# lupoglaz/DeepLocalProteinDocking

Hardware: AMD Instinct MI355X
Metric: pose correlations/sec (48ch x 64^3 pair, 6-degree SOI-sized generated rotation set) (higher is better)
Workload: dtype f32

## Files before the change

### deeplocalproteindocking_amd/csrc/dlpd_k3r.hip

```cpp
#include <dlpd_platform.h>
#include "dlpd_fft.h"
#include "dlpd_internal.h"
#include "dlpd_k3.h"

template <int N> DLPD_D void init_twiddles_k3r(cplx* tw, int tid, int nthreads) {
  for (int k = tid; k < N; k += nthreads) {
    double s, c;
    sincospi(-2.0 * (double)k / (double)N, &s, &c);
    tw[k] = c_make((float)c, (float)s);
  }
}

#ifndef DLPD_K3R_F128
#define DLPD_K3R_F128 4
#endif
#ifndef DLPD_K3R_M160
#define DLPD_K3R_M160 10
#endif
#ifndef DLPD_K3R_TY160
#define DLPD_K3R_TY160 16
#endif
#ifndef DLPD_K3R_PBUF160W
#define DLPD_K3R_PBUF160W 2
#endif
#ifndef DLPD_K3R_DMA_BEHIND_LOADS
#define DLPD_K3R_DMA_BEHIND_LOADS 1
#endif
#ifndef DLPD_K3R_TWREG128
#define DLPD_K3R_TWREG128 1
#endif
#ifndef DLPD_K3R_PBUF128W
#define DLPD_K3R_PBUF128W 2
#endif
#ifndef DLPD_K3R_PBUF128
#define DLPD_K3R_PBUF128 1
#endif
#ifndef DLPD_K3R_PBUF160
#define DLPD_K3R_PBUF160 2
#endif
#ifndef DLPD_K3R_RAWBUF128
#define DLPD_K3R_RAWBUF128 1
#endif
#ifndef DLPD_K3R_FFT_PRIO
#define DLPD_K3R_FFT_PRIO 0
#endif
template <int N> struct K3rWideAbove { static constexpr int value = (N == 160) ? 24 : 32; };
template <int N, bool WIDE> struct K3rCfg;
template <> struct K3rCfg<64, false> { static constexpr int F = 4, M = 4, TY = 16, RAWBUF = 2, PBUF = 1; };
template <> struct K3rCfg<80, false> { static constexpr int F = 5, M = 5, TY = 16, RAWBUF = 2, PBUF = 1; };
template <> struct K3rCfg<128, false> { static constexpr int F = DLPD_K3R_F128, M = 8, TY = 16, RAWBUF = DLPD_K3R_RAWBUF128, PBUF = DLPD_K3R_PBUF128; };
template <> struct K3rCfg<160, false> { static constexpr int F = 5, M = DLPD_K3R_M160, TY = DLPD_K3R_TY160, RAWBUF = 1, PBUF = DLPD_K3R_PBUF160; };
template <> struct K3rCfg<80, true> { static constexpr int F = 5, M = 10, TY = 16, RAWBUF = 1, PBUF = 1; };
template <> struct K3rCfg<128, true> { static constexpr int F = 4, M = 8, TY = 8, RAWBUF = 1, PBUF = DLPD_K3R_PBUF128W; };
template <> struct K3rCfg<160, true> { static constexpr int F = 5, M = 10, TY = 8, RAWBUF = 1, PBUF = DLPD_K3R_PBUF160W; };

#ifdef DLPD_STAMPS
__device__ unsigned long long dlpd_stamps_k3r[32];
extern "C" int dlpd_debug_read_stamps_k3r(unsigned long long* host32) {
  if (hipMemcpyFromSymbol(host32, HIP_SYMBOL(dlpd_stamps_k3r), 32 * sizeof(unsigned long long)) != hipSuccess) return 1;
  unsigned long long z[32] = {0};
  return hipMemcpyToSymbol(HIP_SYMBOL(dlpd_stamps_k3r), z, sizeof(z)) == hipSuccess ? 0 : 1;
}
#endif

#ifndef DLPD_K3R_DC_OPAQUE
#define DLPD_K3R_DC_OPAQUE 0
#endif
#if defined(DLPD_CPU_EMU)
#define DLPD_K3R_KEEP4(q) ((void)0)
#else
#define DLPD_K3R_KEEP4(q) asm("" : "+v"((q).x), "+v"((q).y), "+v"((q).z), "+v"((q).w))
#endif
template <int NPAIR> DLPD_HD int k3r_pair_swz(int k) { return NPAIR == 8 ? ((k & 2) << 1) : 0; }

template <int N> struct K3rFirst { typedef FftPassW<N, N / 8, 1, +1, 8> Pass; };
template <int N, int NPAIR> DLPD_D void k3r_first_pass_load(typename K3rFirst<N>::Pass& ps, int t, int m, const float4* rj) {
  constexpr int NH = N / 2, R1 = N / 8, RH = R1 / 2;
  static_assert(NH % 8 == 0 && R1 % 2 == 0, "bins t + 8r: the first R1/2 direct, the others mirrored");
  const float4* lo = rj + NPAIR * t + (m ^ k3r_pair_swz<NPAIR>(t));
  const float4* hi = rj + NPAIR * (NH - t) + (m ^ k3r_pair_swz<NPAIR>(NH - t));
  {
    float4 q[RH];
#pragma unroll
    for (int r = 0; r < RH; r++) q[r] = lo[NPAIR * 8 * r];
    if (DLPD_K3R_DC_OPAQUE) DLPD_K3R_KEEP4(q[0]);
#pragma unroll
    for (int r = 0; r < RH; r++) {
      const bool dc = (r == 0) && (t == 0);
      ps.v[0][r] = dc ? c_make(q[r].x, q[r].z) : c_make(q[r].x - q[r].w, q[r].y + q[r].z);
    }
  }
  {
    float4 q[RH];
#pragma unroll
    for (int s = 0; s < RH; s++) q[s] = *(hi - NPAIR * 8 * s);
    if (DLPD_K3R_DC_OPAQUE) DLPD_K3R_KEEP4(q[0]);
#pragma unroll
    for (int s = 0; s < RH; s++) {
      const bool ny = (s == 0) && (t == 0);
      ps.v[0][RH + s] = ny ? c_make(q[s].x, q[s].z) : c_make(q[s].x + q[s].w, q[s].z - q[s].y);
    }
  }
  SmallDft<R1, +1>::run(ps.v[0]);
}
template <int N> DLPD_D void k3r_first_pass_store(cplx* S, int rowoff, int t, const typename K3rFirst<N>::Pass& ps) {
  constexpr int R1 = N / 8;
  cplx* P = S + rowoff;
  if constexpr (N == 160) {
#pragma unroll
    for (int r = 0; r < R1; r++) lds_st(P + 21 * t + r, ps.v[0][r]);
  } else if constexpr (N == 80) {
    const RowMid<R1 + 1> md = {rowoff};
    ps.store_blk(S, md, t);
  } else {
    const RowAddr<0> ad = {rowoff};
    ps.store(S, ad, t);
  }
}
template <int N, int NPAIR> DLPD_D void k3r_first_pass(cplx* S, int rowoff, int t, int m, const float4* rj) {
  typename K3rFirst<N>::Pass ps;
  k3r_first_pass_load<N, NPAIR>(ps, t, m, rj);
  k3r_first_pass_store<N>(S, rowoff, t, ps);
}

template <int N> struct K3rTwReg { static constexpr bool value = (N == 128) && (DLPD_K3R_TWREG128 != 0); };
template <int N> struct K3rSecond { typedef FftPassW<N, 8, N / 8, +1, 8> Pass; };
template <int N> DLPD_D void k3r_second_pass(cplx* S, int rowoff, int t, const cplx* tw,
                                             const cplx (&twr)[K3rSecond<N>::Pass::PER][7]) {
  constexpr int R1 = N / 8;
  DLPD_WAVE_SYNC();
  if constexpr (K3rTwReg<N>::value) {
    const RowAddr<0> ad = {rowoff};
    typename K3rSecond<N>::Pass ps;
    ps.load_twr(S, ad, t, twr);
    DLPD_WAVE_SYNC();
    ps.store(S, ad, t);
  } else if constexpr (N == 160) {
    cplx* P = S + rowoff;
    FftPassW<N, 8, 20, +1, 8> ps;
#pragma unroll
    for (int i = 0; i < 3; i++)
      if (t + 8 * i < 20) {
#pragma unroll
        for (int r = 0; r < 8; r++) ps.v[i][r] = lds_ld(P + t + 8 * i + 21 * r);
        ps.twiddle_and_run(i, t + 8 * i, tw);
      }
    DLPD_WAVE_SYNC();
#pragma unroll
    for (int i = 0; i < 3; i++)
      if (t + 8 * i < 20) {
#pragma unroll
        for (int r = 0; r < 8; r++) lds_st(P + t + 8 * i + 21 * r, ps.v[i][r]);
      }
  } else {
    const RowAddr<0> ad = {rowoff};
    FftPassW<N, 8, R1, +1, 8> ps;
    if constexpr (N == 80) {
      const RowMid<R1 + 1> md = {rowoff};
      ps.load_blk(S, md, t, tw);
    } else {
      ps.load(S, ad, t, tw);
    }
    DLPD_WAVE_SYNC();
    ps.store(S, ad, t);
  }
}

template <int N, int HP, int MODE> __global__ void __launch_bounds__(64 * (K3rCfg<N, (HP > K3rWideAbove<N>::value)>::F + K3rCfg<N, (HP > K3rWideAbove<N>::value)>::M))
k_zifft_filter_rs(const cplx* __restrict__ Bw, float* __restrict__ out, int CT, int C, int has_clash, int G,
                  const float* __restrict__ W1t, const float* __restrict__ b1, const float* __restrict__ W2,
                  float b2, int has_clip, float clip, float thr, K3Aux aux, int ntiles, int tpb, K3Cand cd) {
  typedef K3rCfg<N, (HP > K3rWideAbove<N>::value)> Cfg;
  constexpr int F = Cfg::F, M = Cfg::M, TY = Cfg::TY, RAWBUF = Cfg::RAWBUF;
  constexpr int NZ = N / 2 + 1, RS = N + 8, NPAIR = TY / 2, NYT = N / TY;
  constexpr int CPW = 8 / NPAIR;
  constexpr int LPK = 64 / NPAIR;
  constexpr int NFULL = (N / 2) / LPK;
  constexpr int GMAX = F * CPW;
  constexpr int NTM = 64 * M;
  constexpr int EPT = (NPAIR * N) / NTM;
  constexpr int MSTEP = NTM / N;
  constexpr int PBUF = Cfg::PBUF;
  constexpr int PSZ = F * 8 * RS;
  constexpr int RAWC = (PBUF == 2) ? NZ * NPAIR : ((NZ * NPAIR + 63) / 64) * 64;
  static_assert(NPAIR == 8 || NPAIR == 4, "one transform wave = 8 pencils x 8 threads");
  static_assert(EPT >= 1 && EPT * NTM == NPAIR * N && NTM % N == 0, "the filter waves tile the voxels exactly");
  static_assert(NZ * NPAIR == NFULL * 64 + NPAIR, "raw channel = NFULL full DMA instructions + one short one");
  DLPD_DYN_SHARED(cplx, S);
  cplx* tw = S + PBUF * PSZ;
  float4* raw = reinterpret_cast<float4*>(tw + N);
  const int tid = threadIdx.x, lane = tid & 63, wave = tid >> 6;
  const bool is_fft = wave < F;
  const int twave = wave, fwave = wave - F;
  const int t_beg = blockIdx.x * tpb, t_end = (t_beg + tpb < ntiles) ? t_beg + tpb : ntiles;
  if (t_beg >= t_end) return;
  const int plane = t_beg / NYT, plane_x = plane % N, plane_b = plane / N;
  init_twiddles_k3r<N>(tw, tid, 64 * (F + M));
  const unsigned cand_tau = (MODE == 1 && cd.keys) ? *cd.tau : 0u;
  const float clampv = has_clip ? clip : __builtin_inff();

  float4* rawg = raw + twave * CPW * RAWC;
  auto issue_channel = [&](int t, int cb, int buf, int lane) {
    const int ty0 = (t - plane * NYT) * TY, txo = plane_x, tb = plane_b;
#pragma unroll
    for (int j = 0; j < CPW; j++) {
      const int g = twave * CPW + j;
      if (g < G && cb + g < CT) {
        const cplx* src = Bw + (((size_t)tb * CT + cb + DLPD_UNIFORM(g)) * NZ * N + txo) * N + ty0;
        const unsigned lane_off = (unsigned)(((lane / NPAIR) * N * N + 2 * ((lane % NPAIR) ^ k3r_pair_swz<NPAIR>(lane / NPAIR))) * sizeof(cplx));
        const dlpd_lds_t rj = DLPD_LDS_ADDR(rawg + buf * (F * CPW * RAWC) + j * RAWC);
#pragma unroll
        for (int it = 0; it < NFULL; it++) DLPD_GLDS16_SOA(src + (size_t)it * LPK * N * N, lane_off, rj + it * 1024);
        const int mt = lane % NPAIR;
        if (PBUF == 1 || lane < NPAIR) DLPD_GLDS16_SOA(src + (size_t)(N / 2) * N * N, 2 * mt * sizeof(cplx), rj + NFULL * 1024);
      }
    }
  };
  const int tm = 64 * fwave + lane;
  const int zz_ = is_fft ? 0 : tm % N, m0_ = is_fft ? 0 : tm / N;

  if (is_fft) {
    if (DLPD_K3R_FFT_PRIO) DLPD_SET_PRIO(DLPD_K3R_FFT_PRIO);
    issue_channel(t_beg, 0, 0, lane);
  }
  DLPD_LDS_BARRIER();
  DLPD_STAMP_DECL;
  const int ngroups = (CT + G - 1) / G;
  const int nsteps = (t_end - t_beg) * ngroups;
  if (is_fft) {
    int t = t_beg, cbase = 0, rb = 0;
    cplx* P = S;
    cplx twr[K3rSecond<N>::Pass::PER][7];
    if constexpr (K3rTwReg<N>::value) {
      typename K3rSecond<N>::Pass ps0;
      ps0.fetch_twiddles(lane & 7, tw, twr);
    }
#pragma unroll 1
    for (int step = 0; step < nsteps; step++) {
      const int gn = (CT - cbase) < G ? (CT - cbase) : G;
      const bool last_group = cbase + G >= CT;
      const bool mine = twave * CPW < gn;
      int ln = lane;
      if (F + M > 12) DLPD_OPAQUE_V(ln);
      const int tr = ln & 7, qr = ln >> 3;
      if (mine) {
        DLPD_WAIT_VMEM();
        DLPD_WAVE_SYNC();
      }
      DLPD_STAMP(0);
      const int nt = last_group ? t + 1 : t, ncb = last_group ? 0 : cbase + G;
      if (RAWBUF == 2 && nt < t_end) issue_channel(nt, ncb, rb ^ 1, ln);
      if (mine) {
        const int m = qr % NPAIR, j = qr / NPAIR;
        k3r_first_pass<N, NPAIR>(P, (twave * 8 + qr) * RS, tr, m, rawg + rb * (F * CPW * RAWC) + j * RAWC);
        DLPD_WAVE_SYNC();
      }
      DLPD_STAMP(1);
      if constexpr (K3rTwReg<N>::value && DLPD_K3R_DMA_BEHIND_LOADS) {
        const RowAddr<0> ad = {(twave * 8 + qr) * RS};
        typename K3rSecond<N>::Pass ps;
        DLPD_WAVE_SYNC();
        if (mine) ps.load_only(P, ad, tr);
        if (RAWBUF == 1 && nt < t_end) issue_channel(nt, ncb, 0, ln);
        if (mine) {
          ps.run_twr(tr, twr);
          DLPD_WAVE_SYNC();
          ps.store(P, ad, tr);
        }
      } else {
        if (RAWBUF == 1 && nt < t_end) issue_channel(nt, ncb, 0, ln);
        if (mine) k3r_second_pass<N>(P, (twave * 8 + qr) * RS, tr, tw, twr);
      }
      DLPD_STAMP(2);
      if (RAWBUF == 2) rb ^= 1;
      DLPD_LDS_BARRIER();
      DLPD_STAMP(3);
      if (PBUF == 2) {
        P = (P == S) ? S + PSZ : S;
      } else {
        DLPD_LDS_BARRIER();
      }
      DLPD_STAMP(4);
      if (last_group) { cbase = 0; t++; } else cbase += G;
    }
  } else {
    float nrm[EPT * 2];
    float h[EPT * 2][HP];
    cplx vals[PBUF == 2 ? 1 : GMAX][EPT] = {};
    const cplx* P = S;
    int t = t_beg, cbase = 0;
#pragma unroll 1
    for (int step = 0; step < nsteps; step++) {
      const int y0 = (t - plane * NYT) * TY, xo = plane_x, b = plane_b;
      const int gn = (CT - cbase) < G ? (CT - cbase) : G;
      const bool last_group = cbase + G >= CT;
      int zz = zz_, m0 = m0_;
      DLPD_OPAQUE_V(zz);
      DLPD_OPAQUE_V(m0);
      if (cbase == 0) {
        if (MODE == 1 && cd.keys && !cand_tau && tm == 0) cd.count[cd.nb + b] = 1u;
#pragma unroll
        for (int e = 0; e < EPT * 2; e++) nrm[e] = 0.f;
        if (MODE == 1 && aux.C > 0) {
          const int Na = aux.N;
          size_t cstride = (size_t)Na * Na * Na;
          DLPD_OPAQUE_S(cstride);
          const float* ub = aux.p + (size_t)b * HP * cstride + ((size_t)(xo >> 1) * Na + (y0 >> 1)) * Na;
          unsigned lo[EPT];
#pragma unroll
          for (int e = 0; e < EPT; e++) lo[e] = (unsigned)((m0 + e * MSTEP) * Na + (zz >> 1));
#pragma unroll
          for (int e = 0; e < EPT; e++)
#pragma unroll
            for (int j = 0; j < HP; j++) {
              const float v = (ub + (size_t)j * cstride)[lo[e]];
              h[2 * e][j] = v;
              h[2 * e + 1][j] = v;
            }
        } else {
#pragma unroll
          for (int e = 0; e < EPT * 2; e++)
#pragma unroll
            for (int j = 0; j < HP; j++) h[e][j] = b1[j];
        }
      }
      DLPD_STAMP(0);
      DLPD_LDS_BARRIER();
      DLPD_STAMP(1);
      const int gs = (cbase + gn <= C) ? gn : (C - cbase > 0 ? C - cbase : 0);
      if (PBUF == 1) {
#pragma unroll
        for (int g = 0; g < GMAX; g++)
          if (g < gs) {
#pragma unroll
            for (int e = 0; e < EPT; e++) vals[g][e] = S[(g * NPAIR + m0 + e * MSTEP) * RS + pencil_out_pos<N>(zz)];
          }
      }
      if (MODE == 1 && has_clash && cbase + gn > C) {
        const int g = C - cbase;
#pragma unroll
        for (int e = 0; e < EPT; e++) {
          const cplx v = P[(g * NPAIR + m0 + e * MSTEP) * RS + pencil_out_pos<N>(zz)];
          nrm[2 * e] = v.x;
          nrm[2 * e + 1] = v.y;
        }
      }
      if (PBUF == 1) {
        DLPD_LDS_BARRIER();
#pragma unroll
        for (int g = 0; g < GMAX; g++) {
#pragma unroll
          for (int e = 0; e < EPT; e++) { DLPD_SINK_V(vals[g][e].x); DLPD_SINK_V(vals[g][e].y); }
        }
      }
      DLPD_STAMP(2);
      if (PBUF == 2) {
        const cplx* pv = P + (m0 * RS + pencil_out_pos<N>(zz));
        float wcur[HP], wnxt[HP];
        cplx vcur[EPT], vnxt[EPT];
        if (gs > 0) {
#pragma unroll
          for (int j = 0; j < HP; j++) wcur[j] = W1t[(size_t)cbase * HP + j];
#pragma unroll
          for (int e = 0; e < EPT; e++) vcur[e] = pv[e * MSTEP * RS];
#pragma unroll
          for (int j = 0; j < HP; j++) DLPD_SINK_S(wcur[j]);
#pragma unroll
          for (int e = 0; e < EPT; e++) { DLPD_SINK_V(vcur[e].x); DLPD_SINK_V(vcur[e].y); }
        }
#pragma unroll
        for (int g = 0; g < GMAX; g++) {
          if (g < gs) {
            const int gn1 = (g + 1 < gs ? g + 1 : g);
#pragma unroll
            for (int j = 0; j < HP; j++) wnxt[j] = W1t[(size_t)(cbase + gn1) * HP + j];
#pragma unroll
            for (int e = 0; e < EPT; e++) vnxt[e] = pv[(gn1 * NPAIR + e * MSTEP) * RS];
            DLPD_SCHED_FENCE();
#pragma unroll
            for (int e = 0; e < EPT; e++) {
              float v0 = vcur[e].x, v1 = vcur[e].y;
              v0 = DLPD_CLAMP(v0, clampv);
              v1 = DLPD_CLAMP(v1, clampv);
#pragma unroll
              for (int j = 0; j < HP; j++) {
                h[2 * e][j] = fmaf(wcur[j], v0, h[2 * e][j]);
                h[2 * e + 1][j] = fmaf(wcur[j], v1, h[2 * e + 1][j]);
              }
            }
            DLPD_SCHED_FENCE();
#pragma unroll
            for (int j = 0; j < HP; j++) wcur[j] = wnxt[j];
#pragma unroll
            for (int e = 0; e < EPT; e++) vcur[e] = vnxt[e];
          }
        }
        P = (P == S) ? S + PSZ : S;
      } else {
        float wcur[HP], wnxt[HP];
        if (gs > 0) {
#pragma unroll
          for (int j = 0; j < HP; j++) wcur[j] = W1t[(size_t)cbase * HP + j];
#pragma unroll
          for (int j = 0; j < HP; j++) DLPD_SINK_S(wcur[j]);
        }
#pragma unroll
        for (int g = 0; g < GMAX; g++) {
          if (g < gs) {
            const int gn1 = (g + 1 < gs ? g + 1 : g);
#pragma unroll
            for (int j = 0; j < HP; j++) wnxt[j] = W1t[(size_t)(cbase + gn1) * HP + j];
            DLPD_SCHED_FENCE();
#pragma unroll
            for (int e = 0; e < EPT; e++) {
              float v0 = vals[g][e].x, v1 = vals[g][e].y;
              v0 = DLPD_CLAMP(v0, clampv);
              v1 = DLPD_CLAMP(v1, clampv);
#pragma unroll
              for (int j = 0; j < HP; j++) {
                h[2 * e][j] = fmaf(wcur[j], v0, h[2 * e][j]);
                h[2 * e + 1][j] = fmaf(wcur[j], v1, h[2 * e + 1][j]);
              }
            }
            DLPD_SCHED_FENCE();
#pragma unroll
            for (int j = 0; j < HP; j++) wcur[j] = wnxt[j];
          }
        }
      }
      DLPD_STAMP(3);
      if (last_group) {
        if (MODE == 2) {
#pragma unroll
          for (int e = 0; e < EPT; e++) {
            const int m = m0 + e * MSTEP;
#pragma unroll
            for (int u = 0; u < 2; u++) {
              {
#pragma unroll
                for (int j = 0; j < HP; j++)
                  (out + ((((size_t)b * HP + j) * N + xo) * N + y0) * N)[(unsigned)((2 * m + u) * N + zz)] = h[2 * e + u][j];
              }
            }
          }
        } else {
#pragma unroll
          for (int e = 0; e < EPT; e++) {
            const int m = m0 + e * MSTEP;
#pragma unroll
            for (int u = 0; u < 2; u++) {
              float acc = b2;
#pragma unroll
              for (int j = 0; j < HP; j++) acc = fmaf(W2[j], fmaxf(h[2 * e + u][j], 0.f), acc);
              if (has_clash) acc = acc * ((nrm[2 * e + u] < thr) ? 1.0f : 0.0f);
              (out + (((size_t)b * N + xo) * N + y0) * N)[(unsigned)((2 * m + u) * N + zz)] = acc;
              if (cd.keys && cand_tau) k3_emit(cd, cand_tau, b, (unsigned)((xo * N + y0 + 2 * m + u) * N + zz), acc);
            }
          }
        }
        DLPD_STAMP(4);
      }
      if (last_group) { cbase = 0; t++; } else cbase += G;
    }
  }
#ifdef DLPD_STAMPS
  if (lane == 0 && ((is_fft && twave == (DLPD_STAMPS) % F) || (!is_fft && fwave == (DLPD_STAMPS) % M))) {
    const int o = is_fft ? 0 : 16;
    for (int i_ = 0; i_ < 8; i_++) atomicAdd(&dlpd_stamps_k3r[o + i_], st_sum[i_]);
    atomicAdd(&dlpd_stamps_k3r[o + 15], 1ull);
  }
#endif
}

#ifndef DLPD_K3R_TPB_DIV
#define DLPD_K3R_TPB_DIV 1
#endif
static int k3r_group(int CT, int maxg, bool balanced) {
  if (!balanced) return CT < maxg ? CT : maxg;
  const int ng = (CT + maxg - 1) / maxg;
  return (CT + ng - 1) / ng;
}

#ifndef DLPD_K3R_TPB_DIV
#define DLPD_K3R_TPB_DIV 1
#endif
template <int N, int HP, int MODE> static int launch_k3r(const cplx* Bw, float* out, int CT, int C, int has_clash, int nb,
                                                         const float* W1t, const float* b1, const float* W2, float b2,
                                                         int has_clip, float clip, float thr, hipStream_t st, K3Aux aux,
                                                         K3Cand cd) {
  typedef K3rCfg<N, (HP > K3rWideAbove<N>::value)> Cfg;
  constexpr int RS = N + 8, NZ = N / 2 + 1, NPAIR = Cfg::TY / 2, CPW = 8 / NPAIR;
  constexpr int RAWC = (Cfg::PBUF == 2) ? NZ * NPAIR : ((NZ * NPAIR + 63) / 64) * 64;
  const size_t shmem = (size_t)(Cfg::PBUF * Cfg::F * 8 * RS + N) * sizeof(cplx) + (size_t)Cfg::RAWBUF * Cfg::F * CPW * RAWC * 16;
  int rc = dlpd_set_max_dyn_shared((const void*)k_zifft_filter_rs<N, HP, MODE>, shmem);
  if (rc) return rc;
  const int G = k3r_group(CT, Cfg::F * CPW, true);
  const int ntiles = (N / Cfg::TY) * N * nb, tpb = (N / Cfg::TY) / DLPD_K3R_TPB_DIV;
  DLPD_LAUNCH((k_zifft_filter_rs<N, HP, MODE>), dim3((ntiles + tpb - 1) / tpb), dim3(64 * (Cfg::F + Cfg::M)), shmem, st, Bw,
              out, CT, C, has_clash, G, W1t, b1, W2, b2, has_clip, clip, thr, aux, ntiles, tpb, cd);
  return dlpd_check_launch();
}

int dlpd_k3r_supported(int L, int HP, int mode) {
  if (HP != 2 && HP != 4 && HP != 8 && HP != 16 && HP != 24 && HP != 32 && HP != 48) return 0;
  if (mode == 1) return (L == 64 || L == 80) ? 1 : 0;
  if (mode == 2) return (L == 40) ? 1 : 0;
  return 0;
}

template <int N, int MODE> static int k3r_dispatch(int HP, const cplx* Bw, float* out, int CT, int C, int has_clash, int nb,
                                                   const float* W1t, const float* b1, const float* W2, float b2,
                                                   int has_clip, float clip, float thr, hipStream_t st, K3Aux aux, K3Cand cd) {
  switch (HP) {
    case 2: return launch_k3r<N, 2, MODE>(Bw, out, CT, C, has_clash, nb, W1t, b1, W2, b2, has_clip, clip, thr, st, aux, cd);
    case 4: return launch_k3r<N, 4, MODE>(Bw, out, CT, C, has_clash, nb, W1t, b1, W2, b2, has_clip, clip, thr, st, aux, cd);
    case 8: return launch_k3r<N, 8, MODE>(Bw, out, CT, C, has_clash, nb, W1t, b1, W2, b2, has_clip, clip, thr, st, aux, cd);
    case 16: return launch_k3r<N, 16, MODE>(Bw, out, CT, C, has_clash, nb, W1t, b1, W2, b2, has_clip, clip, thr, st, aux, cd);
    case 24: return launch_k3r<N, 24, MODE>(Bw, out, CT, C, has_clash, nb, W1t, b1, W2, b2, has_clip, clip, thr, st, aux, cd);
    case 32: return launch_k3r<N, 32, MODE>(Bw, out, CT, C, has_clash, nb, W1t, b1, W2, b2, has_clip, clip, thr, st, aux, cd);
    case 48: return launch_k3r<N, 48, MODE>(Bw, out, CT, C, has_clash, nb, W1t, b1, W2, b2, has_clip, clip, thr, st, aux, cd);
    default: return DLPD_ERR_UNSUPPORTED;
  }
}

int dlpd_k3r_filter(const cplx* Bw, float* V, int CT, int C, int has_clash, int nb, int L, const float* W1t, int HP,
                    const float* b1, const float* W2, float b2, int has_clip, float clip, float thr, K3Aux aux, K3Cand cd,
                    hipStream_t st) {
  switch (L) {
    case 64: return k3r_dispatch<128, 1>(HP, Bw, V, CT, C, has_clash, nb, W1t, b1, W2, b2, has_clip, clip, thr, st, aux, cd);
    case 80: return k3r_dispatch<160, 1>(HP, Bw, V, CT, C, has_clash, nb, W1t, b1, W2, b2, has_clip, clip, thr, st, aux, cd);
    default: return DLPD_ERR_UNSUPPORTED;
  }
}

int dlpd_k3r_preact(const cplx* Bw, float* pre, int C, int nb, int L, const float* W1rows, int HP, const float* b1,
                    int has_clip, float clip, hipStream_t st) {
  const K3Aux ax = {nullptr, 0, 0, 0};
  const K3Cand cd = {nullptr, nullptr, nullptr, 0, 0};
  switch (L) {
    case 40: return k3r_dispatch<80, 2>(HP, Bw, pre, C, C, 0, nb, W1rows, b1, b1, 0.f, has_clip, clip, 0.f, st, ax, cd);
    default: return DLPD_ERR_UNSUPPORTED;
  }
}
```

Baseline: 6.909 billion.

## Stream tile-channel items flat across FFT waves to fill partial channel groups

Adds a FLAT mode for the N=128 single-pencil-buffer configuration. Instead of processing channels in per-tile groups, where the last group can leave FFT waves idle, the kernel walks a flat (tile, channel) item stream. A step can therefore finish one tile's channels and start the next tile's in the same batch. The filter waves split each step's slots between finishing the current tile's hidden-layer accumulation and seeding the next tile. The aim is to remove idle transform slots at tile boundaries, at the cost of more complex bookkeeping, extra branches and a larger register footprint.

New measurement: 6.407 billion. 0.927x the previous value.

```diff
diff --git a/deeplocalproteindocking_amd/csrc/dlpd_k3r.hip b/deeplocalproteindocking_amd/csrc/dlpd_k3r.hip
--- a/deeplocalproteindocking_amd/csrc/dlpd_k3r.hip
+++ b/deeplocalproteindocking_amd/csrc/dlpd_k3r.hip
@@ -41,18 +41,24 @@
 #ifndef DLPD_K3R_RAWBUF128
 #define DLPD_K3R_RAWBUF128 1
 #endif
+#ifndef DLPD_K3R_FLAT
+#define DLPD_K3R_FLAT 1
+#endif
+#ifndef DLPD_K3R_PPB
+#define DLPD_K3R_PPB 1
+#endif
 #ifndef DLPD_K3R_FFT_PRIO
 #define DLPD_K3R_FFT_PRIO 0
 #endif
 template <int N> struct K3rWideAbove { static constexpr int value = (N == 160) ? 24 : 32; };
 template <int N, bool WIDE> struct K3rCfg;
-template <> struct K3rCfg<64, false> { static constexpr int F = 4, M = 4, TY = 16, RAWBUF = 2, PBUF = 1; };
-template <> struct K3rCfg<80, false> { static constexpr int F = 5, M = 5, TY = 16, RAWBUF = 2, PBUF = 1; };
-template <> struct K3rCfg<128, false> { static constexpr int F = DLPD_K3R_F128, M = 8, TY = 16, RAWBUF = DLPD_K3R_RAWBUF128, PBUF = DLPD_K3R_PBUF128; };
-template <> struct K3rCfg<160, false> { static constexpr int F = 5, M = DLPD_K3R_M160, TY = DLPD_K3R_TY160, RAWBUF = 1, PBUF = DLPD_K3R_PBUF160; };
-template <> struct K3rCfg<80, true> { static constexpr int F = 5, M = 10, TY = 16, RAWBUF = 1, PBUF = 1; };
-template <> struct K3rCfg<128, true> { static constexpr int F = 4, M = 8, TY = 8, RAWBUF = 1, PBUF = DLPD_K3R_PBUF128W; };
-template <> struct K3rCfg<160, true> { static constexpr int F = 5, M = 10, TY = 8, RAWBUF = 1, PBUF = DLPD_K3R_PBUF160W; };
+template <> struct K3rCfg<64, false> { static constexpr int F = 4, M = 4, TY = 16, RAWBUF = 2, PBUF = 1; static constexpr bool FLAT = false; };
+template <> struct K3rCfg<80, false> { static constexpr int F = 5, M = 5, TY = 16, RAWBUF = 2, PBUF = 1; static constexpr bool FLAT = false; };
+template <> struct K3rCfg<128, false> { static constexpr int F = DLPD_K3R_F128, M = 8, TY = 16, RAWBUF = DLPD_K3R_RAWBUF128, PBUF = DLPD_K3R_PBUF128; static constexpr bool FLAT = (DLPD_K3R_FLAT != 0) && (PBUF == 1); };
+template <> struct K3rCfg<160, false> { static constexpr int F = 5, M = DLPD_K3R_M160, TY = DLPD_K3R_TY160, RAWBUF = 1, PBUF = DLPD_K3R_PBUF160; static constexpr bool FLAT = false; };
+template <> struct K3rCfg<80, true> { static constexpr int F = 5, M = 10, TY = 16, RAWBUF = 1, PBUF = 1; static constexpr bool FLAT = false; };
+template <> struct K3rCfg<128, true> { static constexpr int F = 4, M = 8, TY = 8, RAWBUF = 1, PBUF = DLPD_K3R_PBUF128W; static constexpr bool FLAT = false; };
+template <> struct K3rCfg<160, true> { static constexpr int F = 5, M = 10, TY = 8, RAWBUF = 1, PBUF = DLPD_K3R_PBUF160W; static constexpr bool FLAT = false; };
 
 #ifdef DLPD_STAMPS
 __device__ unsigned long long dlpd_stamps_k3r[32];
@@ -166,7 +172,7 @@
   }
 }
 
-template <int N, int HP, int MODE> __global__ void __launch_bounds__(64 * (K3rCfg<N, (HP > K3rWideAbove<N>::value)>::F + K3rCfg<N, (HP > K3rWideAbove<N>::value)>::M))
+template <int N, int HP, int MODE, bool FLAT = false> __global__ void __launch_bounds__(64 * (K3rCfg<N, (HP > K3rWideAbove<N>::value)>::F + K3rCfg<N, (HP > K3rWideAbove<N>::value)>::M))
 k_zifft_filter_rs(const cplx* __restrict__ Bw, float* __restrict__ out, int CT, int C, int has_clash, int G,
                   const float* __restrict__ W1t, const float* __restrict__ b1, const float* __restrict__ W2,
                   float b2, int has_clip, float clip, float thr, K3Aux aux, int ntiles, int tpb, K3Cand cd) {
@@ -200,20 +206,30 @@
   const float clampv = has_clip ? clip : __builtin_inff();
 
   float4* rawg = raw + twave * CPW * RAWC;
+  auto issue_slot = [&](int t, int c, int j, int buf, int lane) {
+    const int pl = FLAT ? t / NYT : plane;
+    const int ty0 = (t - pl * NYT) * TY, txo = FLAT ? pl % N : plane_x, tb = FLAT ? pl / N : plane_b;
+    const cplx* src = Bw + (((size_t)tb * CT + c) * NZ * N + txo) * N + ty0;
+    const unsigned lane_off = (unsigned)(((lane / NPAIR) * N * N + 2 * ((lane % NPAIR) ^ k3r_pair_swz<NPAIR>(lane / NPAIR))) * sizeof(cplx));
+    const dlpd_lds_t rj = DLPD_LDS_ADDR(rawg + buf * (F * CPW * RAWC) + j * RAWC);
+#pragma unroll
+    for (int it = 0; it < NFULL; it++) DLPD_GLDS16_SOA(src + (size_t)it * LPK * N * N, lane_off, rj + it * 1024);
+    const int mt = lane % NPAIR;
+    if (PBUF == 1 || lane < NPAIR) DLPD_GLDS16_SOA(src + (size_t)(N / 2) * N * N, 2 * mt * sizeof(cplx), rj + NFULL * 1024);
+  };
   auto issue_channel = [&](int t, int cb, int buf, int lane) {
-    const int ty0 = (t - plane * NYT) * TY, txo = plane_x, tb = plane_b;
 #pragma unroll
     for (int j = 0; j < CPW; j++) {
       const int g = twave * CPW + j;
-      if (g < G && cb + g < CT) {
-        const cplx* src = Bw + (((size_t)tb * CT + cb + DLPD_UNIFORM(g)) * NZ * N + txo) * N + ty0;
-        const unsigned lane_off = (unsigned)(((lane / NPAIR) * N * N + 2 * ((lane % NPAIR) ^ k3r_pair_swz<NPAIR>(lane / NPAIR))) * sizeof(cplx));
-        const dlpd_lds_t rj = DLPD_LDS_ADDR(rawg + buf * (F * CPW * RAWC) + j * RAWC);
-#pragma unroll
-        for (int it = 0; it < NFULL; it++) DLPD_GLDS16_SOA(src + (size_t)it * LPK * N * N, lane_off, rj + it * 1024);
-        const int mt = lane % NPAIR;
-        if (PBUF == 1 || lane < NPAIR) DLPD_GLDS16_SOA(src + (size_t)(N / 2) * N * N, 2 * mt * sizeof(cplx), rj + NFULL * 1024);
-      }
+      if (g < G && cb + g < CT) issue_slot(t, cb + DLPD_UNIFORM(g), j, buf, lane);
+    }
+  };
+  const int nitems = (t_end - t_beg) * CT;
+  auto issue_items = [&](int i0, int t, int c, int buf, int lane) {
+#pragma unroll
+    for (int j = 0; j < CPW; j++) {
+      if (i0 + j < nitems) issue_slot(t, c, j, buf, lane);
+      if (++c == CT) { c = 0; t++; }
     }
   };
   const int tm = 64 * fwave + lane;
@@ -221,14 +237,16 @@
 
   if (is_fft) {
     if (DLPD_K3R_FFT_PRIO) DLPD_SET_PRIO(DLPD_K3R_FFT_PRIO);
-    issue_channel(t_beg, 0, 0, lane);
+    if constexpr (FLAT) issue_items(DLPD_UNIFORM(twave * CPW), t_beg, DLPD_UNIFORM(twave * CPW), 0, lane);
+    else issue_channel(t_beg, 0, 0, lane);
   }
   DLPD_LDS_BARRIER();
   DLPD_STAMP_DECL;
-  const int ngroups = (CT + G - 1) / G;
-  const int nsteps = (t_end - t_beg) * ngroups;
+  const int ngroups = FLAT ? 0 : (CT + G - 1) / G;
+  const int nsteps = FLAT ? (nitems + GMAX - 1) / GMAX : (t_end - t_beg) * ngroups;
   if (is_fft) {
     int t = t_beg, cbase = 0, rb = 0;
+    int fi = DLPD_UNIFORM(twave * CPW), ft = t_beg, fc = fi;
     cplx* P = S;
     cplx twr[K3rSecond<N>::Pass::PER][7];
     if constexpr (K3rTwReg<N>::value) {
@@ -239,7 +257,7 @@
     for (int step = 0; step < nsteps; step++) {
       const int gn = (CT - cbase) < G ? (CT - cbase) : G;
       const bool last_group = cbase + G >= CT;
-      const bool mine = twave * CPW < gn;
+      const bool mine = FLAT ? fi < nitems : twave * CPW < gn;
       int ln = lane;
       if (F + M > 12) DLPD_OPAQUE_V(ln);
       const int tr = ln & 7, qr = ln >> 3;
@@ -249,7 +267,12 @@
       }
       DLPD_STAMP(0);
       const int nt = last_group ? t + 1 : t, ncb = last_group ? 0 : cbase + G;
-      if (RAWBUF == 2 && nt < t_end) issue_channel(nt, ncb, rb ^ 1, ln);
+      const int nfi = fi + GMAX, nft = (fc + GMAX >= CT) ? ft + 1 : ft, nfc = (fc + GMAX >= CT) ? fc + GMAX - CT : fc + GMAX;
+      auto issue_next = [&](int buf, int l) {
+        if constexpr (FLAT) issue_items(nfi, nft, nfc, buf, l);
+        else if (nt < t_end) issue_channel(nt, ncb, buf, l);
+      };
+      if (RAWBUF == 2) issue_next(rb ^ 1, ln);
       if (mine) {
         const int m = qr % NPAIR, j = qr / NPAIR;
         k3r_first_pass<N, NPAIR>(P, (twave * 8 + qr) * RS, tr, m, rawg + rb * (F * CPW * RAWC) + j * RAWC);
@@ -261,14 +284,14 @@
         typename K3rSecond<N>::Pass ps;
         DLPD_WAVE_SYNC();
         if (mine) ps.load_only(P, ad, tr);
-        if (RAWBUF == 1 && nt < t_end) issue_channel(nt, ncb, 0, ln);
+        if (RAWBUF == 1) issue_next(0, ln);
         if (mine) {
           ps.run_twr(tr, twr);
           DLPD_WAVE_SYNC();
           ps.store(P, ad, tr);
         }
       } else {
-        if (RAWBUF == 1 && nt < t_end) issue_channel(nt, ncb, 0, ln);
+        if (RAWBUF == 1) issue_next(0, ln);
         if (mine) k3r_second_pass<N>(P, (twave * 8 + qr) * RS, tr, tw, twr);
       }
       DLPD_STAMP(2);
@@ -281,105 +304,95 @@
         DLPD_LDS_BARRIER();
       }
       DLPD_STAMP(4);
-      if (last_group) { cbase = 0; t++; } else cbase += G;
+      if constexpr (FLAT) { fi = nfi; ft = nft; fc = nfc; }
+      else if (last_group) { cbase = 0; t++; } else cbase += G;
     }
   } else {
     float nrm[EPT * 2];
     float h[EPT * 2][HP];
     cplx vals[PBUF == 2 ? 1 : GMAX][EPT] = {};
-    const cplx* P = S;
-    int t = t_beg, cbase = 0;
-#pragma unroll 1
-    for (int step = 0; step < nsteps; step++) {
-      const int y0 = (t - plane * NYT) * TY, xo = plane_x, b = plane_b;
-      const int gn = (CT - cbase) < G ? (CT - cbase) : G;
-      const bool last_group = cbase + G >= CT;
-      int zz = zz_, m0 = m0_;
-      DLPD_OPAQUE_V(zz);
-      DLPD_OPAQUE_V(m0);
-      if (cbase == 0) {
-        if (MODE == 1 && cd.keys && !cand_tau && tm == 0) cd.count[cd.nb + b] = 1u;
-#pragma unroll
-        for (int e = 0; e < EPT * 2; e++) nrm[e] = 0.f;
-        if (MODE == 1 && aux.C > 0) {
-          const int Na = aux.N;
-          size_t cstride = (size_t)Na * Na * Na;
-          DLPD_OPAQUE_S(cstride);
-          const float* ub = aux.p + (size_t)b * HP * cstride + ((size_t)(xo >> 1) * Na + (y0 >> 1)) * Na;
-          unsigned lo[EPT];
-#pragma unroll
-          for (int e = 0; e < EPT; e++) lo[e] = (unsigned)((m0 + e * MSTEP) * Na + (zz >> 1));
-#pragma unroll
-          for (int e = 0; e < EPT; e++)
-#pragma unroll
-            for (int j = 0; j < HP; j++) {
-              const float v = (ub + (size_t)j * cstride)[lo[e]];
-              h[2 * e][j] = v;
-              h[2 * e + 1][j] = v;
+    auto init_tile = [&](int t, int zz, int m0) {
+      const int pl = FLAT ? t / NYT : plane;
+      const int y0 = (t - pl * NYT) * TY, xo = FLAT ? pl % N : plane_x, b = FLAT ? pl / N : plane_b;
+      if (MODE == 1 && cd.keys && !cand_tau && tm == 0) cd.count[cd.nb + b] = 1u;
+#pragma unroll
+      for (int e = 0; e < EPT * 2; e++) nrm[e] = 0.f;
+      if (MODE == 1 && aux.C > 0) {
+        const int Na = aux.N;
+        size_t cstride = (size_t)Na * Na * Na;
+        DLPD_OPAQUE_S(cstride);
+        const float* ub = aux.p + (size_t)b * HP * cstride + ((size_t)(xo >> 1) * Na + (y0 >> 1)) * Na;
+        unsigned lo[EPT];
+#pragma unroll
+        for (int e = 0; e < EPT; e++) lo[e] = (unsigned)((m0 + e * MSTEP) * Na + (zz >> 1));
+#pragma unroll
+        for (int e = 0; e < EPT; e++)
+#pragma unroll
+          for (int j = 0; j < HP; j++) {
+            const float v = (ub + (size_t)j * cstride)[lo[e]];
+            h[2 * e][j] = v;
+            h[2 * e + 1][j] = v;
+          }
+      } else {
+#pragma unroll
+        for (int e = 0; e < EPT * 2; e++)
+#pragma unroll
+          for (int j = 0; j < HP; j++) h[e][j] = b1[j];
+      }
+    };
+    auto finish_tile = [&](int t, int zz, int m0) {
+      const int pl = FLAT ? t / NYT : plane;
+      const int y0 = (t - pl * NYT) * TY, xo = FLAT ? pl % N : plane_x, b = FLAT ? pl / N : plane_b;
+      if (MODE == 2) {
+#pragma unroll
+        for (int e = 0; e < EPT; e++) {
+          const int m = m0 + e * MSTEP;
+#pragma unroll
+          for (int u = 0; u < 2; u++) {
+            {
+#pragma unroll
+              for (int j = 0; j < HP; j++)
+                (out + ((((size_t)b * HP + j) * N + xo) * N + y0) * N)[(unsigned)((2 * m + u) * N + zz)] = h[2 * e + u][j];
             }
-        } else {
-#pragma unroll
-          for (int e = 0; e < EPT * 2; e++)
-#pragma unroll
-            for (int j = 0; j < HP; j++) h[e][j] = b1[j];
-        }
-      }
-      DLPD_STAMP(0);
-      DLPD_LDS_BARRIER();
-      DLPD_STAMP(1);
-      const int gs = (cbase + gn <= C) ? gn : (C - cbase > 0 ? C - cbase : 0);
-      if (PBUF == 1) {
-#pragma unroll
-        for (int g = 0; g < GMAX; g++)
-          if (g < gs) {
-#pragma unroll
-            for (int e = 0; e < EPT; e++) vals[g][e] = S[(g * NPAIR + m0 + e * MSTEP) * RS + pencil_out_pos<N>(zz)];
-          }
-      }
-      if (MODE == 1 && has_clash && cbase + gn > C) {
-        const int g = C - cbase;
+          }
+        }
+      } else {
 #pragma unroll
         for (int e = 0; e < EPT; e++) {
-          const cplx v = P[(g * NPAIR + m0 + e * MSTEP) * RS + pencil_out_pos<N>(zz)];
-          nrm[2 * e] = v.x;
-          nrm[2 * e + 1] = v.y;
-        }
-      }
-      if (PBUF == 1) {
-        DLPD_LDS_BARRIER();
+          const int m = m0 + e * MSTEP;
+#pragma unroll
+          for (int u = 0; u < 2; u++) {
+            float acc = b2;
+#pragma unroll
+            for (int j = 0; j < HP; j++) acc = fmaf(W2[j], fmaxf(h[2 * e + u][j], 0.f), acc);
+            if (has_clash) acc = acc * ((nrm[2 * e + u] < thr) ? 1.0f : 0.0f);
+            (out + (((size_t)b * N + xo) * N + y0) * N)[(unsigned)((2 * m + u) * N + zz)] = acc;
+            if (cd.keys && cand_tau) k3_emit(cd, cand_tau, b, (unsigned)((xo * N + y0 + 2 * m + u) * N + zz), acc);
+          }
+        }
+      }
+      DLPD_STAMP(4);
+    };
+    if constexpr (FLAT) {
+      static_assert(PBUF == 1, "the flat stream copies its values out of ONE pencil buffer");
+      auto fold_slots = [&](int lo, int hi, int row0) {
+        float wcur[HP], wnxt[HP];
+        if (lo < hi) {
+#pragma unroll
+          for (int j = 0; j < HP; j++) wcur[j] = W1t[(size_t)(row0 + lo) * HP + j];
+#pragma unroll
+          for (int j = 0; j < HP; j++) DLPD_SINK_S(wcur[j]);
+        }
 #pragma unroll
         for (int g = 0; g < GMAX; g++) {
-#pragma unroll
-          for (int e = 0; e < EPT; e++) { DLPD_SINK_V(vals[g][e].x); DLPD_SINK_V(vals[g][e].y); }
-        }
-      }
-      DLPD_STAMP(2);
-      if (PBUF == 2) {
-        const cplx* pv = P + (m0 * RS + pencil_out_pos<N>(zz));
-        float wcur[HP], wnxt[HP];
-        cplx vcur[EPT], vnxt[EPT];
-        if (gs > 0) {
-#pragma unroll
-          for (int j = 0; j < HP; j++) wcur[j] = W1t[(size_t)cbase * HP + j];
-#pragma unroll
-          for (int e = 0; e < EPT; e++) vcur[e] = pv[e * MSTEP * RS];
-#pragma unroll
-          for (int j = 0; j < HP; j++) DLPD_SINK_S(wcur[j]);
-#pragma unroll
-          for (int e = 0; e < EPT; e++) { DLPD_SINK_V(vcur[e].x); DLPD_SINK_V(vcur[e].y); }
-        }
-#pragma unroll
-        for (int g = 0; g < GMAX; g++) {
-          if (g < gs) {
-            const int gn1 = (g + 1 < gs ? g + 1 : g);
-#pragma unroll
-            for (int j = 0; j < HP; j++) wnxt[j] = W1t[(size_t)(cbase + gn1) * HP + j];
-#pragma unroll
-            for (int e = 0; e < EPT; e++) vnxt[e] = pv[(gn1 * NPAIR + e * MSTEP) * RS];
+          if (g >= lo && g < hi) {
+            const int gn1 = (g + 1 < hi ? g + 1 : g);
+#pragma unroll
+            for (int j = 0; j < HP; j++) wnxt[j] = W1t[(size_t)(row0 + gn1) * HP + j];
             DLPD_SCHED_FENCE();
 #pragma unroll
             for (int e = 0; e < EPT; e++) {
-              float v0 = vcur[e].x, v1 = vcur[e].y;
+              float v0 = vals[g][e].x, v1 = vals[g][e].y;
               v0 = DLPD_CLAMP(v0, clampv);
               v1 = DLPD_CLAMP(v1, clampv);
 #pragma unroll
@@ -391,76 +404,183 @@
             DLPD_SCHED_FENCE();
 #pragma unroll
             for (int j = 0; j < HP; j++) wcur[j] = wnxt[j];
-#pragma unroll
-            for (int e = 0; e < EPT; e++) vcur[e] = vnxt[e];
-          }
-        }
-        P = (P == S) ? S + PSZ : S;
-      } else {
-        float wcur[HP], wnxt[HP];
-        if (gs > 0) {
-#pragma unroll
-          for (int j = 0; j < HP; j++) wcur[j] = W1t[(size_t)cbase * HP + j];
-#pragma unroll
-          for (int j = 0; j < HP; j++) DLPD_SINK_S(wcur[j]);
-        }
+          }
+        }
+      };
+      int t = t_beg, c0 = 0;
+      {
+        int zz = zz_, m0 = m0_;
+        DLPD_OPAQUE_V(zz);
+        DLPD_OPAQUE_V(m0);
+        init_tile(t, zz, m0);
+      }
+#pragma unroll 1
+      for (int step = 0; step < nsteps; step++) {
+        const bool complete = CT - c0 <= GMAX;
+        const int k = complete ? CT - c0 : GMAX;
+        const int kn = (complete && t + 1 < t_end) ? GMAX - k : 0;
+        const int ks = (c0 + k <= C) ? k : (C - c0 > 0 ? C - c0 : 0);
+        int zz = zz_, m0 = m0_;
+        DLPD_OPAQUE_V(zz);
+        DLPD_OPAQUE_V(m0);
+        DLPD_STAMP(0);
+        DLPD_LDS_BARRIER();
+        DLPD_STAMP(1);
+#pragma unroll
+        for (int g = 0; g < GMAX; g++)
+          if (g < ks || (g >= k && g < k + kn)) {
+#pragma unroll
+            for (int e = 0; e < EPT; e++) vals[g][e] = S[(g * NPAIR + m0 + e * MSTEP) * RS + pencil_out_pos<N>(zz)];
+          }
+        if (MODE == 1 && has_clash && complete) {
+          const int g = k - 1;
+#pragma unroll
+          for (int e = 0; e < EPT; e++) {
+            const cplx v = S[(g * NPAIR + m0 + e * MSTEP) * RS + pencil_out_pos<N>(zz)];
+            nrm[2 * e] = v.x;
+            nrm[2 * e + 1] = v.y;
+          }
+        }
+        DLPD_LDS_BARRIER();
 #pragma unroll
         for (int g = 0; g < GMAX; g++) {
-          if (g < gs) {
-            const int gn1 = (g + 1 < gs ? g + 1 : g);
-#pragma unroll
-            for (int j = 0; j < HP; j++) wnxt[j] = W1t[(size_t)(cbase + gn1) * HP + j];
-            DLPD_SCHED_FENCE();
-#pragma unroll
-            for (int e = 0; e < EPT; e++) {
-              float v0 = vals[g][e].x, v1 = vals[g][e].y;
-              v0 = DLPD_CLAMP(v0, clampv);
-              v1 = DLPD_CLAMP(v1, clampv);
-#pragma unroll
-              for (int j = 0; j < HP; j++) {
-                h[2 * e][j] = fmaf(wcur[j], v0, h[2 * e][j]);
-                h[2 * e + 1][j] = fmaf(wcur[j], v1, h[2 * e + 1][j]);
+#pragma unroll
+          for (int e = 0; e < EPT; e++) { DLPD_SINK_V(vals[g][e].x); DLPD_SINK_V(vals[g][e].y); }
+        }
+        DLPD_STAMP(2);
+        fold_slots(0, ks, c0);
+        DLPD_STAMP(3);
+        if (complete) {
+          finish_tile(t, zz, m0);
+          t++;
+          c0 = kn;
+          if (t < t_end) {
+            init_tile(t, zz, m0);
+            fold_slots(k, k + kn, -k);
+          }
+        } else {
+          c0 += GMAX;
+        }
+      }
+    } else {
+      const cplx* P = S;
+      int t = t_beg, cbase = 0;
+#pragma unroll 1
+      for (int step = 0; step < nsteps; step++) {
+        const int gn = (CT - cbase) < G ? (CT - cbase) : G;
+        const bool last_group = cbase + G >= CT;
+        int zz = zz_, m0 = m0_;
+        DLPD_OPAQUE_V(zz);
+        DLPD_OPAQUE_V(m0);
+        if (cbase == 0) init_tile(t, zz, m0);
+        DLPD_STAMP(0);
+        DLPD_LDS_BARRIER();
+        DLPD_STAMP(1);
+        const int gs = (cbase + gn <= C) ? gn : (C - cbase > 0 ? C - cbase : 0);
+        if (PBUF == 1) {
+#pragma unroll
+          for (int g = 0; g < GMAX; g++)
+            if (g < gs) {
+#pragma unroll
+              for (int e = 0; e < EPT; e++) vals[g][e] = S[(g * NPAIR + m0 + e * MSTEP) * RS + pencil_out_pos<N>(zz)];
+            }
+        }
+        if (MODE == 1 && has_clash && cbase + gn > C) {
+          const int g = C - cbase;
+#pragma unroll
+          for (int e = 0; e < EPT; e++) {
+            const cplx v = P[(g * NPAIR + m0 + e * MSTEP) * RS + pencil_out_pos<N>(zz)];
+            nrm[2 * e] = v.x;
+            nrm[2 * e + 1] = v.y;
+          }
+        }
+        if (PBUF == 1) {
+          DLPD_LDS_BARRIER();
+#pragma unroll
+          for (int g = 0; g < GMAX; g++) {
+#pragma unroll
+            for (int e = 0; e < EPT; e++) { DLPD_SINK_V(vals[g][e].x); DLPD_SINK_V(vals[g][e].y); }
+          }
+        }
+        DLPD_STAMP(2);
+        if (PBUF == 2) {
+          const cplx* pv = P + (m0 * RS + pencil_out_pos<N>(zz));
+          float wcur[HP], wnxt[HP];
+          cplx vcur[EPT], vnxt[EPT];
+          if (gs > 0) {
+#pragma unroll
+            for (int j = 0; j < HP; j++) wcur[j] = W1t[(size_t)cbase * HP + j];
+#pragma unroll
+            for (int e = 0; e < EPT; e++) vcur[e] = pv[e * MSTEP * RS];
+#pragma unroll
+            for (int j = 0; j < HP; j++) DLPD_SINK_S(wcur[j]);
+#pragma unroll
+            for (int e = 0; e < EPT; e++) { DLPD_SINK_V(vcur[e].x); DLPD_SINK_V(vcur[e].y); }
+          }
+#pragma unroll
+          for (int g = 0; g < GMAX; g++) {
+            if (g < gs) {
+              const int gn1 = (g + 1 < gs ? g + 1 : g);
+#pragma unroll
+              for (int j = 0; j < HP; j++) wnxt[j] = W1t[(size_t)(cbase + gn1) * HP + j];
+#pragma unroll
+              for (int e = 0; e < EPT; e++) vnxt[e] = pv[(gn1 * NPAIR + e * MSTEP) * RS];
+              DLPD_SCHED_FENCE();
+#pragma unroll
+              for (int e = 0; e < EPT; e++) {
+                float v0 = vcur[e].x, v1 = vcur[e].y;
+                v0 = DLPD_CLAMP(v0, clampv);
+                v1 = DLPD_CLAMP(v1, clampv);
+#pragma unroll
+                for (int j = 0; j < HP; j++) {
+                  h[2 * e][j] = fmaf(wcur[j], v0, h[2 * e][j]);
+                  h[2 * e + 1][j] = fmaf(wcur[j], v1, h[2 * e + 1][j]);
+                }
               }
+              DLPD_SCHED_FENCE();
+#pragma unroll
+              for (int j = 0; j < HP; j++) wcur[j] = wnxt[j];
+#pragma unroll
+              for (int e = 0; e < EPT; e++) vcur[e] = vnxt[e];
             }
-            DLPD_SCHED_FENCE();
-#pragma unroll
-            for (int j = 0; j < HP; j++) wcur[j] = wnxt[j];
-          }
-        }
-      }
-      DLPD_STAMP(3);
-      if (last_group) {
-        if (MODE == 2) {
-#pragma unroll
-          for (int e = 0; e < EPT; e++) {
-            const int m = m0 + e * MSTEP;
-#pragma unroll
-            for (int u = 0; u < 2; u++) {
-              {
-#pragma unroll
-                for (int j = 0; j < HP; j++)
-                  (out + ((((size_t)b * HP + j) * N + xo) * N + y0) * N)[(unsigned)((2 * m + u) * N + zz)] = h[2 * e + u][j];
+          }
+          P = (P == S) ? S + PSZ : S;
+        } else {
+          float wcur[HP], wnxt[HP];
+          if (gs > 0) {
+#pragma unroll
+            for (int j = 0; j < HP; j++) wcur[j] = W1t[(size_t)cbase * HP + j];
+#pragma unroll
+            for (int j = 0; j < HP; j++) DLPD_SINK_S(wcur[j]);
+          }
+#pragma unroll
+          for (int g = 0; g < GMAX; g++) {
+            if (g < gs) {
+              const int gn1 = (g + 1 < gs ? g + 1 : g);
+#pragma unroll
+              for (int j = 0; j < HP; j++) wnxt[j] = W1t[(size_t)(cbase + gn1) * HP + j];
+              DLPD_SCHED_FENCE();
+#pragma unroll
+              for (int e = 0; e < EPT; e++) {
+                float v0 = vals[g][e].x, v1 = vals[g][e].y;
+                v0 = DLPD_CLAMP(v0, clampv);
+                v1 = DLPD_CLAMP(v1, clampv);
+#pragma unroll
+                for (int j = 0; j < HP; j++) {
+                  h[2 * e][j] = fmaf(wcur[j], v0, h[2 * e][j]);
+                  h[2 * e + 1][j] = fmaf(wcur[j], v1, h[2 * e + 1][j]);
+                }
               }
+              DLPD_SCHED_FENCE();
+#pragma unroll
+              for (int j = 0; j < HP; j++) wcur[j] = wnxt[j];
             }
           }
-        } else {
-#pragma unroll
-          for (int e = 0; e < EPT; e++) {
-            const int m = m0 + e * MSTEP;
-#pragma unroll
-            for (int u = 0; u < 2; u++) {
-              float acc = b2;
-#pragma unroll
-              for (int j = 0; j < HP; j++) acc = fmaf(W2[j], fmaxf(h[2 * e + u][j], 0.f), acc);
-              if (has_clash) acc = acc * ((nrm[2 * e + u] < thr) ? 1.0f : 0.0f);
-              (out + (((size_t)b * N + xo) * N + y0) * N)[(unsigned)((2 * m + u) * N + zz)] = acc;
-              if (cd.keys && cand_tau) k3_emit(cd, cand_tau, b, (unsigned)((xo * N + y0 + 2 * m + u) * N + zz), acc);
-            }
-          }
-        }
-        DLPD_STAMP(4);
-      }
-      if (last_group) { cbase = 0; t++; } else cbase += G;
+        }
+        DLPD_STAMP(3);
+        if (last_group) finish_tile(t, zz, m0);
+        if (last_group) { cbase = 0; t++; } else cbase += G;
+      }
     }
   }
 #ifdef DLPD_STAMPS
@@ -492,10 +612,20 @@
   constexpr int RS = N + 8, NZ = N / 2 + 1, NPAIR = Cfg::TY / 2, CPW = 8 / NPAIR;
   constexpr int RAWC = (Cfg::PBUF == 2) ? NZ * NPAIR : ((NZ * NPAIR + 63) / 64) * 64;
   const size_t shmem = (size_t)(Cfg::PBUF * Cfg::F * 8 * RS + N) * sizeof(cplx) + (size_t)Cfg::RAWBUF * Cfg::F * CPW * RAWC * 16;
+  const int ntiles = (N / Cfg::TY) * N * nb, tpb = (N / Cfg::TY) / DLPD_K3R_TPB_DIV;
+  if constexpr (Cfg::FLAT) {
+    const int tpbf = (N / Cfg::TY) * DLPD_K3R_PPB;
+    if (CT >= Cfg::F * CPW) {
+      int rcf = dlpd_set_max_dyn_shared((const void*)k_zifft_filter_rs<N, HP, MODE, true>, shmem);
+      if (rcf) return rcf;
+      DLPD_LAUNCH((k_zifft_filter_rs<N, HP, MODE, true>), dim3((ntiles + tpbf - 1) / tpbf), dim3(64 * (Cfg::F + Cfg::M)), shmem, st,
+                  Bw, out, CT, C, has_clash, 0, W1t, b1, W2, b2, has_clip, clip, thr, aux, ntiles, tpbf, cd);
+      return dlpd_check_launch();
+    }
+  }
   int rc = dlpd_set_max_dyn_shared((const void*)k_zifft_filter_rs<N, HP, MODE>, shmem);
   if (rc) return rc;
   const int G = k3r_group(CT, Cfg::F * CPW, true);
-  const int ntiles = (N / Cfg::TY) * N * nb, tpb = (N / Cfg::TY) / DLPD_K3R_TPB_DIV;
   DLPD_LAUNCH((k_zifft_filter_rs<N, HP, MODE>), dim3((ntiles + tpb - 1) / tpb), dim3(64 * (Cfg::F + Cfg::M)), shmem, st, Bw,
               out, CT, C, has_clash, G, W1t, b1, W2, b2, has_clip, clip, thr, aux, ntiles, tpb, cd);
   return dlpd_check_launch();
```
